# JamesYang007/adelie

Hardware: AMD Instinct MI355X
Metric: lambda-paths/sec (100-lambda grpnet); HBM GB/s vs peak (higher is better)
Workload: dtype f64

## Files before the change

### adelie_amd/_abi.py

```python
import ctypes as C
import os

import numpy as np

F32, F64 = 0, 1
COL_MAJOR, ROW_MAJOR = 0, 1
SCREEN_STRONG, SCREEN_PIVOT = 0, 1
GLM_GAUSSIAN, GLM_BINOMIAL_LOGIT, GLM_GAUSSIAN_IRLS, GLM_MULTINOMIAL, GLM_POISSON, GLM_BINOMIAL_PROBIT = 0, 1, 2, 3, 4, 5
GLM_CALLBACK = 6
GLM_COX = 7
TIE_BRESLOW, TIE_EFRON = 0, 1

POLL_FN = C.CFUNCTYPE(C.c_int, C.c_void_p, C.c_int, C.c_int64, C.c_void_p)
DONE_FN = C.CFUNCTYPE(None, C.c_int32, C.c_int, C.c_void_p)
GLM_GRADIENT_FN = C.CFUNCTYPE(C.c_int, C.c_void_p, C.c_void_p, C.c_void_p)
GLM_HESSIAN_FN = C.CFUNCTYPE(C.c_int, C.c_void_p, C.c_void_p, C.c_void_p, C.c_void_p, C.c_void_p)
GLM_LOSS_FN = C.CFUNCTYPE(C.c_int, C.c_void_p, C.c_void_p, C.POINTER(C.c_double))


CONS_SOLVE_FN = C.CFUNCTYPE(C.c_int, C.c_void_p, C.c_int64, C.c_int64, C.POINTER(C.c_double), C.POINTER(C.c_double),
                           C.POINTER(C.c_double), C.c_double, C.c_double, C.POINTER(C.c_double))
CONS_GRADIENT_FN = C.CFUNCTYPE(C.c_int, C.c_void_p, C.c_int64, C.c_int64, C.POINTER(C.c_double), C.POINTER(C.c_double))
CONS_SOLVE_ZERO_FN = C.CFUNCTYPE(C.c_int, C.c_void_p, C.c_int64, C.c_int64, C.POINTER(C.c_double), C.POINTER(C.c_double))
CONS_DUAL_FN = C.CFUNCTYPE(C.c_int, C.c_void_p, C.c_int64, C.c_int64, C.POINTER(C.c_double))
# ... 198 lines not shown
        + [(n, C.c_int64) for n in ("ns", "nv", "nblk", "n_list")]
        + [(n, C.c_void_p) for n in ("sbegin", "ssize", "voff", "blk_g0", "list", "desc", "Dblk", "gblk", "C")]
        + [("ldc", C.c_int64)]
        + [(n, C.c_void_p) for n in ("xmean", "spen", "vcol", "beta", "g", "is_active", "active_set")]
        + [(n, C.c_double) for n in ("l1", "l2", "newton_tol", "dbeta_tol")]
        + [(n, C.c_int64) for n in ("newton_max_iters", "max_active_size", "mark")]
        + [("rsq", C.c_double), ("resid_sum", C.c_double), ("n_updates", C.c_int64), ("active_size", C.c_int64)]
        + [(n, C.c_void_p) for n in ("dcol", "dlt", "dd", "st_f", "st_i")]
    )


(MULTI_SWEEP, MULTI_STEP, MULTI_FUSED_STEP, MULTI_BLOCK_LISTS, MULTI_EXPAND, MULTI_EXPAND_CROSS, MULTI_AXPY, MULTI_TO_MAJOR,
 MULTI_FROM_MAJOR, MULTI_BATCH_PICK) = range(10)


class MultiPiece(C.Structure):
    _fields_ = (
        [(n, C.c_int64) for n in ("dtype", "mode", "nb", "pb", "K", "icpt")]
        + [("X", C.c_void_p), ("X_elems", C.c_int64), ("x_off", C.c_int64), ("ld", C.c_int64), ("bits", C.c_void_p),
           ("bits_elems", C.c_int64), ("ldb", C.c_int64), ("impute", C.c_void_p), ("v", C.c_void_p), ("v_off", C.c_int64),
           ("out", C.c_void_p), ("w", C.c_void_p), ("r", C.c_void_p), ("dcol", C.c_void_p), ("dlt", C.c_void_p),
           ("n_dcol", C.c_int64), ("nz", C.c_int64), ("cols", C.c_void_p), ("nb_cols", C.c_int64), ("part", C.c_void_p),
           ("part_elems", C.c_int64), ("sign", C.c_double), ("nv", C.c_int64), ("nc", C.c_int64)]
        + [(n, C.c_void_p) for n in ("ulist", "slot", "resp", "slot_c", "resp_c", "C")]
        + [("C_elems", C.c_int64), ("ldc", C.c_int64), ("D", C.c_void_p), ("D_elems", C.c_int64), ("ldd", C.c_int64),
           ("lsel_list", C.c_void_p), ("n_lsel", C.c_int64), ("lsel", C.c_int64)]
    )


HIP_SYMBOLS = [
    "abi_version", "last_error", "device_count", "set_config",
    "design_create_dense", "design_create_sparse", "design_create_csc", "design_create_standardized", "design_adopt_dense_dev", "design_create_snp_unphased",
    "design_create_snp_calldata", "design_create_snp_bed", "design_alias", "design_drop_shadow", "design_shadow_stats", "design_shadow_info", "design_create_slice", "design_create_multi", "design_create_derived", "design_create_concat", "design_create_pieces", "design_impute", "design_destroy", "design_owned_bytes",
    "design_create_one_hot", "design_create_interaction", "design_factor_groups",
    "design_create_convex_relu", "design_create_convex_relu_csc",
    "design_create_snp_phased_ancestry", "design_create_snp_phased_calldata", "design_csc_download", "design_nnz",
    "design_glm_path_losses", "design_multi_path_losses", "design_cox_path_losses", "design_batch_stats", "design_rows", "design_cols", "design_dtype",
    "design_device", "design_stream",
    "design_cmul", "design_ctmul", "design_bmul", "design_btmul", "design_bmul_cols", "design_btmul_cols", "design_mul", "design_mul_batch", "design_cov",
    "design_sq_mul", "design_sp_tmul",
    "design_create_cov_dense", "design_create_cov_csc", "design_create_cov_lazy", "design_cov_bmul", "design_cov_mul", "design_cov_mul_batch", "design_cov_to_dense", "gaussian_cov_solve",
    "glm_cox_create", "glm_cox_destroy", "glm_cox_eval",
    "grpnet_solve", "grpnet_solve_many", "result_destroy", "result_size", "result_copy", "result_scalar", "result_error", "result_sync",
    "bench_sweep", "filter_sweep_test", "block_build_test", "group_piece_test", "multi_piece_test", "cov_piece_test",
    "css_cov_solve", "css_result_destroy", "css_result_size", "css_result_copy", "css_result_scalar", "css_result_error",
    "bvls_solve", "bvls_result_destroy", "bvls_result_size", "bvls_result_copy", "bvls_result_scalar", "bvls_result_error",
    "design_create_constraint_dense", "design_adopt_constraint_dense_dev", "design_create_constraint_csc", "constraint_op",
    "pinball_solve", "pinball_result_destroy", "pinball_result_size", "pinball_result_copy", "pinball_result_scalar",
    "pinball_result_error",
    "qp_full_solve",
]


def np_dtype(code):
    return np.float64 if code == F64 else np.float32


def dtype_code(dtype):
    dtype = np.dtype(dtype)
# ... 98 lines not shown
        sig("design_cov_bmul", ci, [vp, vp, i64, vp, vp, i64, vp])
        sig("design_cov_mul", ci, [vp, vp, vp, i64, vp])
        sig("design_cov_mul_batch", ci, [vp, i64, vp, vp, vp, vp, vp])
        sig("design_cov_to_dense", ci, [vp, i64, i64, vp])
        sig("result_destroy", ci, [vp])
        sig("result_size", i64, [vp, ci])
        sig("result_copy", ci, [vp, ci, vp, i64])
        sig("result_scalar", dbl, [vp, ci])
        sig("result_error", C.c_char_p, [vp])
        sig("result_sync", ci, [vp])
        sig("bench_sweep", ci, [vp, i64, p(dbl)])
        sig("filter_sweep_test", ci, [vp, vp, vp, dbl, vp, vp, i64, vp, vp, i64, vp, dbl, vp, vp, vp])
        sig("block_build_test", ci, [vp, ci, i64, vp, vp, i64, vp, i64, vp, ci, i64, ci, vp, i64, vp, i64, vp])
        sig("group_piece_test", ci, [p(GroupPiece), vp])
        sig("multi_piece_test", ci, [p(MultiPiece), vp])
        sig("cov_piece_test", ci, [vp, ci, vp, i64, i64, i64, i64, dbl, vp, vp, vp, i64, vp])
        sig("css_cov_solve", ci, [vp, p(CssArgs), p(vp)])
        sig("css_result_destroy", ci, [vp])
        sig("css_result_size", i64, [vp, ci])
        sig("css_result_copy", ci, [vp, ci, vp, i64])
        sig("css_result_scalar", dbl, [vp, ci])
        sig("css_result_error", C.c_char_p, [vp])
        sig("bvls_solve", ci, [vp, p(BvlsArgs), p(vp)])
        sig("bvls_result_destroy", ci, [vp])
        sig("bvls_result_size", i64, [vp, ci])
        sig("bvls_result_copy", ci, [vp, ci, vp, i64])
        sig("bvls_result_scalar", dbl, [vp, ci])
        sig("bvls_result_error", C.c_char_p, [vp])
        sig("design_create_constraint_dense", ci, [vp, i64, i64, ci, ci, ci, p(vp)])
        sig("design_adopt_constraint_dense_dev", ci, [vp, i64, i64, ci, ci, ci, p(vp)])
# ... 55 lines not shown
```

### adelie_amd/csrc/kernels.hpp

```cpp
#pragma once
#include <hip/hip_runtime.h>
#include <cstdint>
#include "gram_shape.hpp"
#include "multi_shape.hpp"
#include "relu_shape.hpp"
#include "relu_sparse_shape.hpp"
#include "shadow_kind_host.hpp"
#include "pieces_host.hpp"

namespace ahip {

template <class T>
struct DenseView {
    const T* X;
    int64_t n, p, ld;
};
struct SnpView {
    const uint8_t* bits;
    int64_t n, p, ldb;
};

template <class T>
struct PiecesView {
    const void* base[kMaxPieces];
// ... 443 lines not shown
int launch_panel_step(const DenseView<T>& X, const T* w, T* r, const int32_t* dcol, const T* dlt, const int32_t* nz_dev,
                      const int32_t* cols, int nb, T* part, hipStream_t s);
template <class T>
struct StepTail {
    int32_t* counter;
    int32_t base;
    T* g;
    const T* rsum;
    const T* xm;
};
template <class T>
int launch_panel_step_snp(const SnpView& X, const T* impute, const T* w, T* r, const int32_t* dcol, const T* dlt,
                          const int32_t* nz_dev, const int32_t* cols, int nb, T* part, hipStream_t s,
                          const StepTail<T>* tail = nullptr, bool* tailed = nullptr);
int64_t panel_part_elems(int64_t n);
template <class T>
void launch_la_open_from_grad(const T* grad, const int32_t* cols, int nb, T* g, const T* rsum_src, T* rsum_out, hipStream_t s);
template <class T>
void launch_panel_reduce(const T* part, int nslices, int nb, const int32_t* cols, const T* rsum_dev, const T* xm_by_col,
                         T* gblk, hipStream_t s);
template <class T>
void launch_panel_reduce_ld(const T* part, int64_t part_ld, int nslices, int nb, const int32_t* cols, const T* rsum_dev,
                            const T* xm_by_col, T* gblk, hipStream_t s);
template <class T>
int launch_panel_fused(const CdBlkParams<T>& sp, int j, const DenseView<T>& X, const T* w, T* r, const int32_t* dcol,
                       const T* dlt, const int32_t* nz_dev, const int32_t* cols, int nb, T* part, bool tr, hipStream_t s);
template <class T>
int launch_panel_fused_snp(const CdBlkParams<T>& sp, int j, const SnpView& X, const T* impute, const T* w, T* r,
                           const int32_t* dcol, const T* dlt, const int32_t* nz_dev, const int32_t* cols, int nb, T* part,
                           bool tr, hipStream_t s);
// ... 221 lines not shown
```

### adelie_amd/csrc/kernels_cd_panel.hip

```cpp
#include "kernels.hpp"
#include "accessors.hpp"
#include "wavered.hpp"
#include "blk_solve_body.hpp"
#include "grp_solve_body.hpp"

namespace ahip {

namespace {

constexpr int PB = 128;
constexpr int PT = 256;

template <class T, int VEC>
struct RawDense { Pack<T, VEC> v; };
struct RawSnp { unsigned byte; };

template <class T, int VEC>
__device__ __forceinline__ RawDense<T, VEC> praw(const DenseAcc<T>& X, int64_t j, int64_t i, int64_t n, bool full) {
    RawDense<T, VEC> r;
    const T* col = X.colptr(j);
    if constexpr (VEC == 1) {
        const T x = col[(full || i < n) ? i : 0];
        r.v.v[0] = (full || i < n) ? x : T(0);
    } else {
        using V = typename VecOf<T>::type;
        static_assert(VEC == VecOf<T>::N, "dense vector width");
// ... 24 lines not shown
template <class T, int VEC>
__device__ __forceinline__ Pack<T, VEC> pdecode(const SnpAcc<T>& X, const RawSnp& r, int64_t j, int64_t i, int64_t n) {
    Pack<T, VEC> o;
    const T imp = X.impute[j];
#pragma unroll
    for (int e = 0; e < VEC; ++e) {
        const unsigned c = (r.byte >> (2 * e)) & 3u;
        o.v[e] = (i + e < n) ? (c == 3u ? imp : T(c)) : T(0);
    }
    return o;
}
template <class T, class Acc, int VEC> struct RawOf;
template <class T, int VEC> struct RawOf<T, DenseAcc<T>, VEC> { using type = RawDense<T, VEC>; };
template <class T, int VEC> struct RawOf<T, SnpAcc<T>, VEC> { using type = RawSnp; };

template <class T, class Acc, int VEC, bool FULL, bool WGRED = false>
__device__ __forceinline__ void panel_step_body(const Acc& X, int64_t n, const T* __restrict__ w, T* __restrict__ r,
                                                const int32_t* __restrict__ dcol, const T* __restrict__ dlt, int nz,
                                                const int32_t* __restrict__ cols, int nb, T* __restrict__ part,
                                                int64_t part_ld, T (*red)[64 * VEC], T* wrs, int tid, int64_t slice) {
    constexpr int U = 16;
    using Raw = typename RawOf<T, Acc, VEC>::type;
    const int lane = tid & 63;
    const int wv = __builtin_amdgcn_readfirstlane(tid >> 6);
    const int64_t i = slice * (64 * VEC) + int64_t(lane) * VEC;
    const bool full = FULL ? true : (i + VEC <= n);

    constexpr int UB = 8;
    Raw xb[UB];
    int jb[UB];
    if (nb > 0) {
#pragma unroll
        for (int u = 0; u < UB; ++u) jb[u] = cols[min(wv + 4 * u, nb - 1)];
#pragma unroll
        for (int u = 0; u < UB; ++u) xb[u] = praw<T, VEC>(X, jb[u], i, n, full);
    }

    if (nz > 0) {
        T acc[VEC];
#pragma unroll
        for (int e = 0; e < VEC; ++e) acc[e] = T(0);
        for (int m0 = wv; m0 < nz; m0 += 4 * U) {
// ... 5 lines not shown
                const int m = m0 + 4 * u;
                ja[u] = dcol[min(m, nz - 1)];
                cf[u] = m < nz ? dlt[min(m, nz - 1)] : T(0);
            }
#pragma unroll
            for (int u = 0; u < U; ++u) xa[u] = praw<T, VEC>(X, ja[u], i, n, full);
#pragma unroll
            for (int u = 0; u < U; ++u) {
                const Pack<T, VEC> xx = pdecode<T, VEC>(X, xa[u], ja[u], i, n);
#pragma unroll
                for (int e = 0; e < VEC; ++e) acc[e] = fma(cf[u], xx.v[e], acc[e]);
            }
        }
#pragma unroll
        for (int e = 0; e < VEC; ++e) red[wv][lane * VEC + e] = acc[e];
        __syncthreads();
        if (wv == 0) {
#pragma unroll
            for (int e = 0; e < VEC; ++e) {
                const int q = lane * VEC + e;
                T wr = T(0);
                if (FULL || i + e < n) {
                    const T rr = r[i + e] - ((red[0][q] + red[1][q]) + (red[2][q] + red[3][q]));
                    r[i + e] = rr;
                    wr = w[i + e] * rr;
                }
                wrs[q] = wr;
            }
        }
    } else if (wv == 0) {
#pragma unroll
        for (int e = 0; e < VEC; ++e) wrs[lane * VEC + e] = (FULL || i + e < n) ? w[i + e] * r[i + e] : T(0);
    }
    if (nb <= 0) return;
    __syncthreads();

    T wr[VEC];
#pragma unroll
    for (int e = 0; e < VEC; ++e) wr[e] = wrs[lane * VEC + e];
    for (int c0 = wv; c0 < nb; c0 += 4 * UB) {
        if (c0 != wv) {
#pragma unroll
            for (int u = 0; u < UB; ++u) jb[u] = cols[min(c0 + 4 * u, nb - 1)];
#pragma unroll
            for (int u = 0; u < UB; ++u) xb[u] = praw<T, VEC>(X, jb[u], i, n, full);
        }
        T pu[UB];
#pragma unroll
        for (int u = 0; u < UB; ++u) {
            const Pack<T, VEC> xx = pdecode<T, VEC>(X, xb[u], jb[u], i, n);
            T sacc = T(0);
#pragma unroll
            for (int e = 0; e < VEC; ++e) sacc = fma(xx.v[e], wr[e], sacc);
            pu[u] = sacc;
        }
        static_assert(UB == 8, "reduce8");
        const T tot = reduce8(pu, lane);
        if (lane < UB && c0 + 4 * lane < nb) {
            if constexpr (WGRED) red[0][c0 + 4 * lane] = tot;
            else part[part_ld > 0 ? int64_t(c0 + 4 * lane) * part_ld + slice : slice * PB + (c0 + 4 * lane)] = tot;
        }
    }
}

template <class T, class Acc, int VEC>
__global__ __launch_bounds__(PT, (VEC >= 16 ? 2 : 4)) void panel_step_kernel(Acc X, int64_t n, const T* __restrict__ w, T* __restrict__ r,
                                                        const int32_t* __restrict__ dcol, const T* __restrict__ dlt,
                                                        const int32_t* __restrict__ nz_dev,
                                                        const int32_t* __restrict__ cols, int nb, T* __restrict__ part,
                                                        int64_t part_ld) {
    constexpr int RS = 64 * VEC;
    __shared__ T red[4][RS];
    __shared__ T wrs[RS];
    const int nz = nz_dev[0];
    if ((int64_t(blockIdx.x) + 1) * RS <= n)
        panel_step_body<T, Acc, VEC, true>(X, n, w, r, dcol, dlt, nz, cols, nb, part, part_ld, red, wrs, threadIdx.x, blockIdx.x);
    else
        panel_step_body<T, Acc, VEC, false>(X, n, w, r, dcol, dlt, nz, cols, nb, part, part_ld, red, wrs, threadIdx.x, blockIdx.x);
}

constexpr int S16_RS = 1024;
constexpr int S16_NSUB = 2;

template <class T>
__device__ __forceinline__ T reduce16(const T (&v)[16], int lane) {
    const bool b0 = lane & 1, b1 = lane & 2, b2 = lane & 4, b3 = lane & 8;
    T a[8], c[4], d[2];
#pragma unroll
    for (int m = 0; m < 8; ++m) {
        const T keep = b0 ? v[2 * m + 1] : v[2 * m], send = b0 ? v[2 * m] : v[2 * m + 1];
        a[m] = keep + pdpp<0xB1>(send);
    }
#pragma unroll
// ... 205 lines not shown
#pragma unroll
            for (int u = 0; u < 4; ++u)
                v[u] = (k0 + 64 * u < nwg) ? __hip_atomic_load(pc + k0 + 64 * u, __ATOMIC_RELAXED, __HIP_MEMORY_SCOPE_AGENT) : T(0);
#pragma unroll
            for (int u = 0; u < 4; ++u) sacc += v[u];
        }
        sacc = wave_sum64(sacc);
        if (lane == 0) {
            T g = sacc;
            if (tail.xm) g -= tail.rsum[0] * tail.xm[cols[c]];
            tail.g[c] = g;
        }
    }
}

constexpr int FS = 4;
template <class T>
constexpr size_t fused_lds() {
    return blk_solve_lds_la<T>() > size_t(148) * 1024 ? blk_solve_lds_la<T>() : size_t(148) * 1024;
}
template <class T, class Acc, int VEC>
__device__ __forceinline__ void fused_step_part(char* smem_raw, const Acc& X, int64_t n, const T* __restrict__ w,
                                                T* __restrict__ r, const int32_t* __restrict__ dcol,
                                                const T* __restrict__ dlt, const int32_t* __restrict__ nz_dev,
                                                const int32_t* __restrict__ cols, int nb, T* __restrict__ part,
                                                int64_t part_ld, int fsa, bool coh = false) {
    constexpr int RS = 64 * VEC;
    const int sub = threadIdx.x >> 8, tid = threadIdx.x & 255;
    T* base = reinterpret_cast<T*>(smem_raw) + size_t(sub) * 5 * RS;
    T (*red)[RS] = reinterpret_cast<T (*)[RS]>(base);
    T* wrs = base + 4 * RS;
    const int nz = nz_dev[0];
    static_assert(RS >= PB || VEC == 1, "a slice's LDS row holds the block's column partials");
    const int64_t grp = int64_t(blockIdx.x) - 1;
    const int64_t slice = grp * fsa + sub;
    if constexpr (RS >= PB) {
        if (sub >= fsa) {
            if (nz > 0) __syncthreads();
            if (nb <= 0) return;
            __syncthreads();
            if (tid < PB) red[0][tid] = T(0);
        } else if ((grp + 1) * fsa * RS <= n) {
            panel_step_body<T, Acc, VEC, true, true>(X, n, w, r, dcol, dlt, nz, cols, nb, part, part_ld, red, wrs, tid, slice);
        } else {
            panel_step_body<T, Acc, VEC, false, true>(X, n, w, r, dcol, dlt, nz, cols, nb, part, part_ld, red, wrs, tid, slice);
        }
        if (nb <= 0) return;
        __syncthreads();
        if (threadIdx.x < nb) {
            const T* b0 = reinterpret_cast<const T*>(smem_raw);
            const int c = threadIdx.x;
            const T tot = (b0[c] + b0[size_t(5) * RS + c]) + (b0[size_t(10) * RS + c] + b0[size_t(15) * RS + c]);
            T* dst = part + (part_ld > 0 ? int64_t(c) * part_ld + grp : grp * PB + c);
            if (coh) __hip_atomic_store(dst, tot, __ATOMIC_RELAXED, __HIP_MEMORY_SCOPE_AGENT);
            else *dst = tot;
        }
    } else {
        const int64_t slice4 = grp * FS + sub;
        if ((grp + 1) * FS * RS <= n)
            panel_step_body<T, Acc, VEC, true>(X, n, w, r, dcol, dlt, nz, cols, nb, part, part_ld, red, wrs, tid, slice4);
        else
            panel_step_body<T, Acc, VEC, false>(X, n, w, r, dcol, dlt, nz, cols, nb, part, part_ld, red, wrs, tid, slice4);
    }
}

inline int fused_fsa(int64_t ns) {
    if ((ns + 3) / 4 > 250) return 4;
    if (ns <= 250) return 1;
    if ((ns + 1) / 2 <= 250) return 2;
    return 4;
}

template <class T, class Acc, int VEC>
__global__ __launch_bounds__(256 * FS) void panel_fused_kernel(CdBlkParams<T> sp, int j, Acc X, int64_t n,
                                                              const T* __restrict__ w, T* __restrict__ r,
                                                              const int32_t* __restrict__ dcol, const T* __restrict__ dlt,
                                                              const int32_t* __restrict__ nz_dev,
                                                              const int32_t* __restrict__ cols, int nb,
                                                              T* __restrict__ part, int64_t part_ld, int fsa) {
    extern __shared__ __attribute__((aligned(16))) char smem_raw[];
    constexpr int RS = 64 * VEC;
    if (blockIdx.x == 0) {
        if (j < 0) {
            if (threadIdx.x == 0 && sp.part_rsum) {
                const T v = sp.part_rsum[0];
                sp.rsum_out[0] = v;
                sp.rsum_out[1] = v;
            }
            return;
        }
        blk_solve_la_body<T>(sp, j, smem_raw, threadIdx.x);
        return;
    }
    fused_step_part<T, Acc, VEC>(smem_raw, X, n, w, r, dcol, dlt, nz_dev, cols, nb, part, part_ld, fsa);
}

template <class T>
__global__ __launch_bounds__(PT) void panel_reduce_kernel(const T* __restrict__ part, int64_t part_ld, int nslices,
                                                          const int32_t* __restrict__ cols,
                                                          const T* __restrict__ rsum, const T* __restrict__ xm_by_col,
                                                          T* __restrict__ gblk) {
    __shared__ T red[4];
    const int c = blockIdx.x, tid = threadIdx.x, lane = tid & 63, wv = tid >> 6;
    const T* pc = part + int64_t(c) * part_ld;
    T s = T(0);
    for (int k = tid; k < nslices; k += PT) s += pc[k];
    s = wave_sum64(s);
    if (lane == 0) red[wv] = s;
    __syncthreads();
// ... 10 lines not shown
    if (a >= cnt) return;
    T v = vars[a];
    if (center) v -= xm[a] * xm[a];
    vars[a] = v > T(0) ? v : T(0);
}

__global__ void gather_i32_kernel(const int32_t* __restrict__ src, const int32_t* __restrict__ idx, int cnt,
                                  int32_t* __restrict__ out) {
    const int a = blockIdx.x * blockDim.x + threadIdx.x;
    if (a < cnt) out[a] = src[idx[a]];
}

template <class T, class Acc, int VEC>
int step_launch(const Acc& acc, int64_t n, const T* w, T* r, const int32_t* dcol, const T* dlt, const int32_t* nz_dev,
                const int32_t* cols, int nb, T* part, hipStream_t s) {
    constexpr int RS = 64 * VEC;
    const int64_t ns = (n + RS - 1) / RS;
    hipLaunchKernelGGL((panel_step_kernel<T, Acc, VEC>), dim3((unsigned)ns), dim3(PT), 0, s, acc, n, w, r, dcol, dlt,
                       nz_dev, cols, nb, part, ns);
    return int(ns);
}

template <class T, class Acc, int VEC>
__global__ __launch_bounds__(256 * FS) void panel_fused_grp_kernel(CdGrpBlkParams<T> sp, int j, Acc X, int64_t n,
                                                                  const T* __restrict__ w, T* __restrict__ r,
                                                                  const int32_t* __restrict__ dcol,
                                                                  const T* __restrict__ dlt,
                                                                  const int32_t* __restrict__ nz_dev,
                                                                  const int32_t* __restrict__ cols, int nb,
                                                                  T* __restrict__ part, int64_t part_ld, int fsa) {
    extern __shared__ __attribute__((aligned(16))) char smem_raw[];
    constexpr int RS = 64 * VEC;
// ... 52 lines not shown
            sp.tail_g[c] = g;
        }
        if (threadIdx.x == 0) {
            const int d = __hip_atomic_fetch_add(sp.tail_counter + 1, 1, __ATOMIC_RELAXED, __HIP_MEMORY_SCOPE_AGENT);
            if (d == NT - 1) {
                __hip_atomic_store(sp.tail_counter + 1, 0, __ATOMIC_RELAXED, __HIP_MEMORY_SCOPE_AGENT);
                __hip_atomic_store(sp.tail_counter, 0, __ATOMIC_RELAXED, __HIP_MEMORY_SCOPE_AGENT);
            }
        }
    }
}

template <class T, class Acc, int VEC>
int fused_grp_launch(const CdGrpBlkParams<T>& sp, int j, const Acc& acc, int64_t n, const T* w, T* r, const int32_t* dcol,
                     const T* dlt, const int32_t* nz_dev, const int32_t* cols, int nb, T* part, bool tr, hipStream_t s) {
    constexpr int RS = 64 * VEC;
    const int64_t ns = (n + RS - 1) / RS;
    const int fsa = (64 * VEC >= PB) ? fused_fsa(ns) : FS;
    const int64_t nwg = (ns + fsa - 1) / fsa;
    const int64_t part_ld = (64 * VEC >= PB) ? nwg : nwg * FS;
    static bool attr_done = false;
    if (!attr_done) {
        (void)hipFuncSetAttribute(reinterpret_cast<const void*>(panel_fused_grp_kernel<T, Acc, VEC>),
                                  hipFuncAttributeMaxDynamicSharedMemorySize, int(grp_solve_lds_total<T>()));
        attr_done = true;
    }
    hipLaunchKernelGGL((panel_fused_grp_kernel<T, Acc, VEC>), dim3((unsigned)(nwg + 1)), dim3(256 * FS),
                       grp_solve_lds_total<T>(), s, sp, j, acc, n, w, r, dcol, dlt, nz_dev, cols, nb, part,
                       tr ? int64_t(0) : part_ld, fsa);
    return int(part_ld);
}

template <class T, class Acc, int VEC>
int fused_launch(const CdBlkParams<T>& sp, int j, const Acc& acc, int64_t n, const T* w, T* r, const int32_t* dcol,
                 const T* dlt, const int32_t* nz_dev, const int32_t* cols, int nb, T* part, bool tr, hipStream_t s) {
    constexpr int RS = 64 * VEC;
    const int64_t ns = (n + RS - 1) / RS;
    const int fsa = (64 * VEC >= PB) ? fused_fsa(ns) : FS;
    const int64_t nwg = (ns + fsa - 1) / fsa;
    const int64_t part_ld = (64 * VEC >= PB) ? nwg : nwg * FS;
    static bool attr_done = false;
    if (!attr_done) {
        (void)hipFuncSetAttribute(reinterpret_cast<const void*>(panel_fused_kernel<T, Acc, VEC>),
                                  hipFuncAttributeMaxDynamicSharedMemorySize, int(fused_lds<T>()));
        attr_done = true;
    }
    hipLaunchKernelGGL((panel_fused_kernel<T, Acc, VEC>), dim3((unsigned)(nwg + 1)), dim3(256 * FS),
                       fused_lds<T>(), s, sp, j, acc, n, w, r, dcol, dlt, nz_dev, cols, nb, part,
                       tr ? int64_t(0) : part_ld, fsa);
    return int(part_ld);
}

}

template <class T>
int launch_panel_fused(const CdBlkParams<T>& sp, int j, const DenseView<T>& X, const T* w, T* r, const int32_t* dcol,
                       const T* dlt, const int32_t* nz_dev, const int32_t* cols, int nb, T* part, bool tr, hipStream_t s) {
    DenseAcc<T> acc{X.X, X.ld};
    constexpr int V = VecOf<T>::N;
    const bool vecok = (X.ld % V == 0) && ((reinterpret_cast<uintptr_t>(X.X) % 16) == 0);
    if (vecok) return fused_launch<T, DenseAcc<T>, V>(sp, j, acc, X.n, w, r, dcol, dlt, nz_dev, cols, nb, part, tr, s);
    return fused_launch<T, DenseAcc<T>, 1>(sp, j, acc, X.n, w, r, dcol, dlt, nz_dev, cols, nb, part, tr, s);
}
template <class T>
int launch_panel_fused_snp(const CdBlkParams<T>& sp, int j, const SnpView& X, const T* impute, const T* w, T* r,
                           const int32_t* dcol, const T* dlt, const int32_t* nz_dev, const int32_t* cols, int nb, T* part,
                           bool tr, hipStream_t s) {
    SnpAcc<T> acc{X.bits, X.ldb, impute};
    return fused_launch<T, SnpAcc<T>, 4>(sp, j, acc, X.n, w, r, dcol, dlt, nz_dev, cols, nb, part, tr, s);
}

template <class T>
int launch_panel_fused_grp(const CdGrpBlkParams<T>& sp, int j, const DenseView<T>& X, const T* w, T* r, const int32_t* dcol,
                           const T* dlt, const int32_t* nz_dev, const int32_t* cols, int nb, T* part, bool tr, hipStream_t s) {
    DenseAcc<T> acc{X.X, X.ld};
// ... 18 lines not shown
    if (c < nb) g[c] = grad[cols[c]];
    if (c == 0 && rsum_src) {
        const T v = rsum_src[0];
        rsum_out[0] = v;
        rsum_out[1] = v;
    }
}
}
template <class T>
void launch_la_open_from_grad(const T* grad, const int32_t* cols, int nb, T* g, const T* rsum_src, T* rsum_out, hipStream_t s) {
    hipLaunchKernelGGL((la_open_kernel<T>), dim3(1), dim3(PB), 0, s, grad, cols, nb, g, rsum_src, rsum_out);
}
template void launch_la_open_from_grad<double>(const double*, const int32_t*, int, double*, const double*, double*, hipStream_t);
template void launch_la_open_from_grad<float>(const float*, const int32_t*, int, float*, const float*, float*, hipStream_t);

int64_t panel_part_elems(int64_t n) { return int64_t(PB) * ((n + 63) / 64) + 16; }

template <class T>
int launch_panel_step(const DenseView<T>& X, const T* w, T* r, const int32_t* dcol, const T* dlt, const int32_t* nz_dev,
                      const int32_t* cols, int nb, T* part, hipStream_t s) {
    DenseAcc<T> acc{X.X, X.ld};
    constexpr int V = VecOf<T>::N;
    const bool vecok = (X.ld % V == 0) && ((reinterpret_cast<uintptr_t>(X.X) % 16) == 0);
    if (vecok) return step_launch<T, DenseAcc<T>, V>(acc, X.n, w, r, dcol, dlt, nz_dev, cols, nb, part, s);
    return step_launch<T, DenseAcc<T>, 1>(acc, X.n, w, r, dcol, dlt, nz_dev, cols, nb, part, s);
}

template <class T>
int launch_panel_step_snp(const SnpView& X, const T* impute, const T* w, T* r, const int32_t* dcol, const T* dlt,
                          const int32_t* nz_dev, const int32_t* cols, int nb, T* part, hipStream_t s, const StepTail<T>* tail,
                          bool* tailed) {
// ... 69 lines not shown
```

### adelie_amd/csrc/solver.hip

```cpp
#include "common.hpp"
#include "design_ops.hpp"
#include "filter_host.hpp"
#include "screen_reads_host.hpp"
#include "cox.hpp"

#include <algorithm>
#include <cstring>
#include <exception>
#include <type_traits>
#include <chrono>
#include <condition_variable>
#include <mutex>
#include <thread>
#include <cmath>
#include <cstdio>
#include <cstdlib>
#include <limits>
#include <numeric>
#include <unordered_set>

namespace ahip {
void set_last_error(const std::string& s);
double g_hessian_min = 1e-24;
double g_dbeta_tol = 1e-12;
// ... 1453 lines not shown
            up(dr, &scale, 1);
            if (a->w) up(dw, static_cast<const T*>(a->w), pb);
            launch_batch_pick<T>(dv.p, pb, int(K), int(a->lsel), dr.p, a->w ? dw.p : nullptr, dout.p, s);
            std::vector<T> h(static_cast<size_t>(pb));
            finish(a->out, h, dout.p);
        };
        if (a->dtype == ADELIE_HIP_F64) body(double{});
        else body(float{});
    } catch (const std::exception& e) {
        set_last_error(e.what());
        return 1;
    }
    return 0;
}

int adelie_hip_cov_piece_test(adelie_hip_design* A, int what, const int32_t* vcol, int64_t nv, int64_t pos0, int64_t N, int64_t ldc,
                              double sentinel, const void* v, const int32_t* cols, const void* coef, int64_t count, void* out) {
    try {
        if (!A || !out) throw make_core_error("bad arguments.");
        if (!A->cov) throw make_core_error("A must be a covariance matrix (matrix.dense(method=\"cov\")).");
        const int64_t p = A->p;
        const bool gather = what == ADELIE_HIP_COV_PIECE_GATHER;
        if (!gather && what != ADELIE_HIP_COV_PIECE_GRAD) throw make_core_error("unknown piece.");
        const int32_t* list = gather ? vcol : cols;
        const int64_t n_list = gather ? nv : count;
        if (gather && (!vcol || nv < 1 || nv > p || pos0 < 0 || N < 1 || pos0 + N != nv || ldc < nv || ldc > (int64_t(1) << 20)))
            throw make_core_error("GATHER: vcol (nv), 1 <= nv <= p, pos0 + N == nv and nv <= ldc are required.");
        if (!gather && (!v || count < 0 || count > p || (count > 0 && (!cols || !coef))))
            throw make_core_error("GRAD: v (p), cols and coef (count), 0 <= count <= p are required.");
        std::vector<uint8_t> seen(size_t(p), 0);
// ... 46 lines not shown
```

### include/adelie_hip.h

```cpp
#ifndef ADELIE_HIP_H
#define ADELIE_HIP_H

#include <stdint.h>

#ifdef __cplusplus
extern "C" {
#endif

#define ADELIE_HIP_ABI_VERSION 14

enum adelie_hip_dtype { ADELIE_HIP_F32 = 0, ADELIE_HIP_F64 = 1 };
enum adelie_hip_order { ADELIE_HIP_COL_MAJOR = 0, ADELIE_HIP_ROW_MAJOR = 1 };
enum adelie_hip_screen_rule { ADELIE_HIP_SCREEN_STRONG = 0, ADELIE_HIP_SCREEN_PIVOT = 1 };
enum adelie_hip_glm_kind {
    ADELIE_HIP_GLM_GAUSSIAN = 0,
    ADELIE_HIP_GLM_BINOMIAL_LOGIT = 1,
    ADELIE_HIP_GLM_GAUSSIAN_IRLS = 2,
    ADELIE_HIP_GLM_POISSON = 4,
    ADELIE_HIP_GLM_BINOMIAL_PROBIT = 5,
    ADELIE_HIP_GLM_CALLBACK = 6,
    ADELIE_HIP_GLM_COX = 7,
    ADELIE_HIP_GLM_MULTINOMIAL = 3
};

// ... 516 lines not shown
    int64_t nv, nc;
    int32_t* ulist;
    int32_t* slot;
    int32_t* resp;
    const int32_t* slot_c;
    const int32_t* resp_c;
    const void* C;
    int64_t C_elems, ldc;
    void* D;
    int64_t D_elems, ldd;
    const int64_t* lsel_list;
    int64_t n_lsel, lsel;
} adelie_hip_multi_piece;
int adelie_hip_multi_piece_test(const adelie_hip_multi_piece* a, int64_t* info);

enum adelie_hip_cov_piece { ADELIE_HIP_COV_PIECE_GATHER = 0, ADELIE_HIP_COV_PIECE_GRAD = 1 };
int adelie_hip_cov_piece_test(adelie_hip_design* A, int what, const int32_t* vcol, int64_t nv, int64_t pos0, int64_t N, int64_t ldc,
                              double sentinel, const void* v, const int32_t* cols, const void* coef, int64_t count, void* out);

enum adelie_hip_qp_full_kind { ADELIE_HIP_QP_FULL_NNQP = 0, ADELIE_HIP_QP_FULL_LASSO = 1, ADELIE_HIP_QP_FULL_PINBALL = 2 };
enum adelie_hip_qp_full_status { ADELIE_HIP_QP_FULL_OK = 0, ADELIE_HIP_QP_FULL_MAX_ITERS = 1 };
typedef struct adelie_hip_qp_full_args {
    int32_t            kind;
    int32_t            dtype;
    int32_t            device;
    int32_t            _pad0;
    int64_t            n_problems;
    const int64_t*     d;
    const void* const* quad;
    const uint8_t*     quad_is_dev;
// ... 18 lines not shown
```

Measured before the change: 5.015.

## Prefetch residual/weights and software-pipeline column loads in dense panel step kernels

For dense designs with vector width at least 2, the panel step body now loads r and w into registers before the reduction. It swaps __syncthreads for a bare LDS-wait plus s_barrier. When nb spans exactly four unroll rounds, it double-buffers column loads with scheduling barriers so global loads overlap the FMA reductions. It also moves the panel shape math into a shared header and adds a panel piece test entry point. The cost is higher register pressure and a special-case code path, and the lighter barrier relies on only LDS ordering being needed.

After: 5.039, median of 3. Within noise of the previous version (+0.5%).

```diff
diff --git a/adelie_amd/_abi.py b/adelie_amd/_abi.py
--- a/adelie_amd/_abi.py
+++ b/adelie_amd/_abi.py
@@ -236,6 +236,13 @@
  MULTI_FROM_MAJOR, MULTI_BATCH_PICK) = range(10)
 
 
+class PanelPiece(C.Structure):
+    _fields_ = [("mode", C.c_int64), ("d", C.c_void_p), ("row_off", C.c_int64), ("w", C.c_void_p), ("r", C.c_void_p),
+                ("dcol", C.c_void_p), ("dlt", C.c_void_p), ("n_dcol", C.c_int64), ("nz", C.c_int64), ("cols", C.c_void_p),
+                ("nb", C.c_int64), ("part", C.c_void_p), ("part_elems", C.c_int64), ("slice_major", C.c_int64), ("g", C.c_void_p),
+                ("g_elems", C.c_int64), ("xm", C.c_void_p), ("resid_sum", C.c_double)]
+
+
 class MultiPiece(C.Structure):
     _fields_ = (
         [(n, C.c_int64) for n in ("dtype", "mode", "nb", "pb", "K", "icpt")]
@@ -264,7 +271,7 @@
     "design_create_cov_dense", "design_create_cov_csc", "design_create_cov_lazy", "design_cov_bmul", "design_cov_mul", "design_cov_mul_batch", "design_cov_to_dense", "gaussian_cov_solve",
     "glm_cox_create", "glm_cox_destroy", "glm_cox_eval",
     "grpnet_solve", "grpnet_solve_many", "result_destroy", "result_size", "result_copy", "result_scalar", "result_error", "result_sync",
-    "bench_sweep", "filter_sweep_test", "block_build_test", "group_piece_test", "multi_piece_test", "cov_piece_test",
+    "bench_sweep", "filter_sweep_test", "block_build_test", "group_piece_test", "multi_piece_test", "panel_piece_test", "cov_piece_test",
     "css_cov_solve", "css_result_destroy", "css_result_size", "css_result_copy", "css_result_scalar", "css_result_error",
     "bvls_solve", "bvls_result_destroy", "bvls_result_size", "bvls_result_copy", "bvls_result_scalar", "bvls_result_error",
     "design_create_constraint_dense", "design_adopt_constraint_dense_dev", "design_create_constraint_csc", "constraint_op",
@@ -393,6 +400,7 @@
         sig("block_build_test", ci, [vp, ci, i64, vp, vp, i64, vp, i64, vp, ci, i64, ci, vp, i64, vp, i64, vp])
         sig("group_piece_test", ci, [p(GroupPiece), vp])
         sig("multi_piece_test", ci, [p(MultiPiece), vp])
+        sig("panel_piece_test", ci, [p(PanelPiece), vp])
         sig("cov_piece_test", ci, [vp, ci, vp, i64, i64, i64, i64, dbl, vp, vp, vp, i64, vp])
         sig("css_cov_solve", ci, [vp, p(CssArgs), p(vp)])
         sig("css_result_destroy", ci, [vp])
diff --git a/adelie_amd/csrc/kernels.hpp b/adelie_amd/csrc/kernels.hpp
--- a/adelie_amd/csrc/kernels.hpp
+++ b/adelie_amd/csrc/kernels.hpp
@@ -3,6 +3,7 @@
 #include <cstdint>
 #include "gram_shape.hpp"
 #include "multi_shape.hpp"
+#include "panel_shape.hpp"
 #include "relu_shape.hpp"
 #include "relu_sparse_shape.hpp"
 #include "shadow_kind_host.hpp"
@@ -481,6 +482,7 @@
                           const int32_t* nz_dev, const int32_t* cols, int nb, T* part, hipStream_t s,
                           const StepTail<T>* tail = nullptr, bool* tailed = nullptr);
 int64_t panel_part_elems(int64_t n);
+template <class T> int panel_step_vec(const DenseView<T>& X);
 template <class T>
 void launch_la_open_from_grad(const T* grad, const int32_t* cols, int nb, T* g, const T* rsum_src, T* rsum_out, hipStream_t s);
 template <class T>
diff --git a/adelie_amd/csrc/kernels_cd_panel.hip b/adelie_amd/csrc/kernels_cd_panel.hip
--- a/adelie_amd/csrc/kernels_cd_panel.hip
+++ b/adelie_amd/csrc/kernels_cd_panel.hip
@@ -1,15 +1,17 @@
 #include "kernels.hpp"
+#include <type_traits>
 #include "accessors.hpp"
 #include "wavered.hpp"
 #include "blk_solve_body.hpp"
 #include "grp_solve_body.hpp"
+#include "panel_shape.hpp"
 
 namespace ahip {
 
 namespace {
 
-constexpr int PB = 128;
-constexpr int PT = 256;
+constexpr int PB = kPanelB;
+constexpr int PT = kPanelThreads;
 
 template <class T, int VEC>
 struct RawDense { Pack<T, VEC> v; };
@@ -64,7 +66,9 @@
 template <class T, int VEC> struct RawOf<T, DenseAcc<T>, VEC> { using type = RawDense<T, VEC>; };
 template <class T, int VEC> struct RawOf<T, SnpAcc<T>, VEC> { using type = RawSnp; };
 
-template <class T, class Acc, int VEC, bool FULL, bool WGRED = false>
+__device__ __forceinline__ void lds_barrier() { asm volatile("s_waitcnt lgkmcnt(0)\n\ts_barrier" ::: "memory"); }
+
+template <class T, class Acc, int VEC, bool FULL, bool WGRED = false, bool STREAM = false>
 __device__ __forceinline__ void panel_step_body(const Acc& X, int64_t n, const T* __restrict__ w, T* __restrict__ r,
                                                 const int32_t* __restrict__ dcol, const T* __restrict__ dlt, int nz,
                                                 const int32_t* __restrict__ cols, int nb, T* __restrict__ part,
@@ -76,6 +80,17 @@
     const int64_t i = slice * (64 * VEC) + int64_t(lane) * VEC;
     const bool full = FULL ? true : (i + VEC <= n);
 
+    T rp[VEC], wp[VEC];
+    if constexpr (STREAM) {
+        if (wv == 0) {
+#pragma unroll
+            for (int e = 0; e < VEC; ++e) {
+                const int64_t q = (FULL || i + e < n) ? i + e : 0;
+                rp[e] = r[q];
+                wp[e] = w[q];
+            }
+        }
+    }
     constexpr int UB = 8;
     Raw xb[UB];
     int jb[UB];
@@ -111,41 +126,39 @@
         }
 #pragma unroll
         for (int e = 0; e < VEC; ++e) red[wv][lane * VEC + e] = acc[e];
-        __syncthreads();
+        if constexpr (STREAM) lds_barrier();
+        else __syncthreads();
         if (wv == 0) {
 #pragma unroll
             for (int e = 0; e < VEC; ++e) {
                 const int q = lane * VEC + e;
                 T wr = T(0);
                 if (FULL || i + e < n) {
-                    const T rr = r[i + e] - ((red[0][q] + red[1][q]) + (red[2][q] + red[3][q]));
+                    const T r0 = STREAM ? rp[e] : r[i + e];
+                    const T rr = r0 - ((red[0][q] + red[1][q]) + (red[2][q] + red[3][q]));
                     r[i + e] = rr;
-                    wr = w[i + e] * rr;
+                    wr = (STREAM ? wp[e] : w[i + e]) * rr;
                 }
                 wrs[q] = wr;
             }
         }
     } else if (wv == 0) {
 #pragma unroll
-        for (int e = 0; e < VEC; ++e) wrs[lane * VEC + e] = (FULL || i + e < n) ? w[i + e] * r[i + e] : T(0);
+        for (int e = 0; e < VEC; ++e)
+            wrs[lane * VEC + e] = (FULL || i + e < n) ? (STREAM ? wp[e] * rp[e] : w[i + e] * r[i + e]) : T(0);
     }
     if (nb <= 0) return;
-    __syncthreads();
+    if constexpr (STREAM) lds_barrier();
+    else __syncthreads();
 
     T wr[VEC];
 #pragma unroll
     for (int e = 0; e < VEC; ++e) wr[e] = wrs[lane * VEC + e];
-    for (int c0 = wv; c0 < nb; c0 += 4 * UB) {
-        if (c0 != wv) {
-#pragma unroll
-            for (int u = 0; u < UB; ++u) jb[u] = cols[min(c0 + 4 * u, nb - 1)];
-#pragma unroll
-            for (int u = 0; u < UB; ++u) xb[u] = praw<T, VEC>(X, jb[u], i, n, full);
-        }
+    const auto consume = [&](const Raw(&x)[UB], const int(&j)[UB], int c0) {
         T pu[UB];
 #pragma unroll
         for (int u = 0; u < UB; ++u) {
-            const Pack<T, VEC> xx = pdecode<T, VEC>(X, xb[u], jb[u], i, n);
+            const Pack<T, VEC> xx = pdecode<T, VEC>(X, x[u], j[u], i, n);
             T sacc = T(0);
 #pragma unroll
             for (int e = 0; e < VEC; ++e) sacc = fma(xx.v[e], wr[e], sacc);
@@ -157,6 +170,43 @@
             if constexpr (WGRED) red[0][c0 + 4 * lane] = tot;
             else part[part_ld > 0 ? int64_t(c0 + 4 * lane) * part_ld + slice : slice * PB + (c0 + 4 * lane)] = tot;
         }
+    };
+    if constexpr (STREAM) {
+        if (wv + 3 * 4 * UB < nb && wv + 4 * 4 * UB >= nb) {
+            Raw x1[UB];
+            int j1[UB], j2[UB], j3[UB];
+#pragma unroll
+            for (int u = 0; u < UB; ++u) {
+                j1[u] = cols[min(wv + 4 * UB + 4 * u, nb - 1)];
+                j2[u] = cols[min(wv + 8 * UB + 4 * u, nb - 1)];
+                j3[u] = cols[min(wv + 12 * UB + 4 * u, nb - 1)];
+            }
+#pragma unroll
+            for (int u = 0; u < UB; ++u) x1[u] = praw<T, VEC>(X, j1[u], i, n, full);
+            __builtin_amdgcn_sched_barrier(0);
+            consume(xb, jb, wv);
+            __builtin_amdgcn_sched_barrier(0);
+#pragma unroll
+            for (int u = 0; u < UB; ++u) xb[u] = praw<T, VEC>(X, j2[u], i, n, full);
+            __builtin_amdgcn_sched_barrier(0);
+            consume(x1, j1, wv + 4 * UB);
+            __builtin_amdgcn_sched_barrier(0);
+#pragma unroll
+            for (int u = 0; u < UB; ++u) x1[u] = praw<T, VEC>(X, j3[u], i, n, full);
+            __builtin_amdgcn_sched_barrier(0);
+            consume(xb, j2, wv + 8 * UB);
+            consume(x1, j3, wv + 12 * UB);
+            return;
+        }
+    }
+    for (int c0 = wv; c0 < nb; c0 += 4 * UB) {
+        if (c0 != wv) {
+#pragma unroll
+            for (int u = 0; u < UB; ++u) jb[u] = cols[min(c0 + 4 * u, nb - 1)];
+#pragma unroll
+            for (int u = 0; u < UB; ++u) xb[u] = praw<T, VEC>(X, jb[u], i, n, full);
+        }
+        consume(xb, jb, c0);
     }
 }
 
@@ -169,11 +219,19 @@
     constexpr int RS = 64 * VEC;
     __shared__ T red[4][RS];
     __shared__ T wrs[RS];
-    const int nz = nz_dev[0];
-    if ((int64_t(blockIdx.x) + 1) * RS <= n)
-        panel_step_body<T, Acc, VEC, true>(X, n, w, r, dcol, dlt, nz, cols, nb, part, part_ld, red, wrs, threadIdx.x, blockIdx.x);
-    else
-        panel_step_body<T, Acc, VEC, false>(X, n, w, r, dcol, dlt, nz, cols, nb, part, part_ld, red, wrs, threadIdx.x, blockIdx.x);
+    if constexpr (std::is_same<Acc, DenseAcc<T>>::value && VEC >= 2) {
+        const int nz = nz_dev[0];
+        if ((int64_t(blockIdx.x) + 1) * RS <= n)
+            panel_step_body<T, Acc, VEC, true, false, true>(X, n, w, r, dcol, dlt, nz, cols, nb, part, part_ld, red, wrs, threadIdx.x, blockIdx.x);
+        else
+            panel_step_body<T, Acc, VEC, false, false, true>(X, n, w, r, dcol, dlt, nz, cols, nb, part, part_ld, red, wrs, threadIdx.x, blockIdx.x);
+    } else {
+        const int nz = nz_dev[0];
+        if ((int64_t(blockIdx.x) + 1) * RS <= n)
+            panel_step_body<T, Acc, VEC, true>(X, n, w, r, dcol, dlt, nz, cols, nb, part, part_ld, red, wrs, threadIdx.x, blockIdx.x);
+        else
+            panel_step_body<T, Acc, VEC, false>(X, n, w, r, dcol, dlt, nz, cols, nb, part, part_ld, red, wrs, threadIdx.x, blockIdx.x);
+    }
 }
 
 constexpr int S16_RS = 1024;
@@ -409,12 +467,12 @@
     }
 }
 
-constexpr int FS = 4;
+constexpr int FS = kPanelFS;
 template <class T>
 constexpr size_t fused_lds() {
     return blk_solve_lds_la<T>() > size_t(148) * 1024 ? blk_solve_lds_la<T>() : size_t(148) * 1024;
 }
-template <class T, class Acc, int VEC>
+template <class T, class Acc, int VEC, bool STREAM = false>
 __device__ __forceinline__ void fused_step_part(char* smem_raw, const Acc& X, int64_t n, const T* __restrict__ w,
                                                 T* __restrict__ r, const int32_t* __restrict__ dcol,
                                                 const T* __restrict__ dlt, const int32_t* __restrict__ nz_dev,
@@ -436,9 +494,15 @@
             __syncthreads();
             if (tid < PB) red[0][tid] = T(0);
         } else if ((grp + 1) * fsa * RS <= n) {
-            panel_step_body<T, Acc, VEC, true, true>(X, n, w, r, dcol, dlt, nz, cols, nb, part, part_ld, red, wrs, tid, slice);
+            if constexpr (STREAM && std::is_same<Acc, DenseAcc<T>>::value)
+                panel_step_body<T, Acc, VEC, true, true, true>(X, n, w, r, dcol, dlt, nz, cols, nb, part, part_ld, red, wrs, tid, slice);
+            else
+                panel_step_body<T, Acc, VEC, true, true>(X, n, w, r, dcol, dlt, nz, cols, nb, part, part_ld, red, wrs, tid, slice);
         } else {
-            panel_step_body<T, Acc, VEC, false, true>(X, n, w, r, dcol, dlt, nz, cols, nb, part, part_ld, red, wrs, tid, slice);
+            if constexpr (STREAM && std::is_same<Acc, DenseAcc<T>>::value)
+                panel_step_body<T, Acc, VEC, false, true, true>(X, n, w, r, dcol, dlt, nz, cols, nb, part, part_ld, red, wrs, tid, slice);
+            else
+                panel_step_body<T, Acc, VEC, false, true>(X, n, w, r, dcol, dlt, nz, cols, nb, part, part_ld, red, wrs, tid, slice);
         }
         if (nb <= 0) return;
         __syncthreads();
@@ -457,13 +521,6 @@
         else
             panel_step_body<T, Acc, VEC, false>(X, n, w, r, dcol, dlt, nz, cols, nb, part, part_ld, red, wrs, tid, slice4);
     }
-}
-
-inline int fused_fsa(int64_t ns) {
-    if ((ns + 3) / 4 > 250) return 4;
-    if (ns <= 250) return 1;
-    if ((ns + 1) / 2 <= 250) return 2;
-    return 4;
 }
 
 template <class T, class Acc, int VEC>
@@ -487,7 +544,7 @@
         blk_solve_la_body<T>(sp, j, smem_raw, threadIdx.x);
         return;
     }
-    fused_step_part<T, Acc, VEC>(smem_raw, X, n, w, r, dcol, dlt, nz_dev, cols, nb, part, part_ld, fsa);
+    fused_step_part<T, Acc, VEC, true>(smem_raw, X, n, w, r, dcol, dlt, nz_dev, cols, nb, part, part_ld, fsa);
 }
 
 template <class T>
@@ -528,8 +585,7 @@
 template <class T, class Acc, int VEC>
 int step_launch(const Acc& acc, int64_t n, const T* w, T* r, const int32_t* dcol, const T* dlt, const int32_t* nz_dev,
                 const int32_t* cols, int nb, T* part, hipStream_t s) {
-    constexpr int RS = 64 * VEC;
-    const int64_t ns = (n + RS - 1) / RS;
+    const int64_t ns = panel_step_shape(n, VEC).slices;
     hipLaunchKernelGGL((panel_step_kernel<T, Acc, VEC>), dim3((unsigned)ns), dim3(PT), 0, s, acc, n, w, r, dcol, dlt,
                        nz_dev, cols, nb, part, ns);
     return int(ns);
@@ -612,11 +668,9 @@
 template <class T, class Acc, int VEC>
 int fused_grp_launch(const CdGrpBlkParams<T>& sp, int j, const Acc& acc, int64_t n, const T* w, T* r, const int32_t* dcol,
                      const T* dlt, const int32_t* nz_dev, const int32_t* cols, int nb, T* part, bool tr, hipStream_t s) {
-    constexpr int RS = 64 * VEC;
-    const int64_t ns = (n + RS - 1) / RS;
-    const int fsa = (64 * VEC >= PB) ? fused_fsa(ns) : FS;
-    const int64_t nwg = (ns + fsa - 1) / fsa;
-    const int64_t part_ld = (64 * VEC >= PB) ? nwg : nwg * FS;
+    const PanelStepShape sh = panel_fused_shape(n, VEC);
+    const int fsa = sh.fsa;
+    const int64_t nwg = sh.wgs, part_ld = sh.part_n;
     static bool attr_done = false;
     if (!attr_done) {
         (void)hipFuncSetAttribute(reinterpret_cast<const void*>(panel_fused_grp_kernel<T, Acc, VEC>),
@@ -632,11 +686,9 @@
 template <class T, class Acc, int VEC>
 int fused_launch(const CdBlkParams<T>& sp, int j, const Acc& acc, int64_t n, const T* w, T* r, const int32_t* dcol,
                  const T* dlt, const int32_t* nz_dev, const int32_t* cols, int nb, T* part, bool tr, hipStream_t s) {
-    constexpr int RS = 64 * VEC;
-    const int64_t ns = (n + RS - 1) / RS;
-    const int fsa = (64 * VEC >= PB) ? fused_fsa(ns) : FS;
-    const int64_t nwg = (ns + fsa - 1) / fsa;
-    const int64_t part_ld = (64 * VEC >= PB) ? nwg : nwg * FS;
+    const PanelStepShape sh = panel_fused_shape(n, VEC);
+    const int fsa = sh.fsa;
+    const int64_t nwg = sh.wgs, part_ld = sh.part_n;
     static bool attr_done = false;
     if (!attr_done) {
         (void)hipFuncSetAttribute(reinterpret_cast<const void*>(panel_fused_kernel<T, Acc, VEC>),
@@ -652,11 +704,19 @@
 }
 
 template <class T>
+int panel_step_vec(const DenseView<T>& X) {
+    constexpr int V = VecOf<T>::N;
+    return ((X.ld % V == 0) && ((reinterpret_cast<uintptr_t>(X.X) % 16) == 0)) ? V : 1;
+}
+template int panel_step_vec<double>(const DenseView<double>&);
+template int panel_step_vec<float>(const DenseView<float>&);
+
+template <class T>
 int launch_panel_fused(const CdBlkParams<T>& sp, int j, const DenseView<T>& X, const T* w, T* r, const int32_t* dcol,
                        const T* dlt, const int32_t* nz_dev, const int32_t* cols, int nb, T* part, bool tr, hipStream_t s) {
     DenseAcc<T> acc{X.X, X.ld};
     constexpr int V = VecOf<T>::N;
-    const bool vecok = (X.ld % V == 0) && ((reinterpret_cast<uintptr_t>(X.X) % 16) == 0);
+    const bool vecok = panel_step_vec<T>(X) == V;
     if (vecok) return fused_launch<T, DenseAcc<T>, V>(sp, j, acc, X.n, w, r, dcol, dlt, nz_dev, cols, nb, part, tr, s);
     return fused_launch<T, DenseAcc<T>, 1>(sp, j, acc, X.n, w, r, dcol, dlt, nz_dev, cols, nb, part, tr, s);
 }
@@ -705,7 +765,7 @@
 template void launch_la_open_from_grad<double>(const double*, const int32_t*, int, double*, const double*, double*, hipStream_t);
 template void launch_la_open_from_grad<float>(const float*, const int32_t*, int, float*, const float*, float*, hipStream_t);
 
-int64_t panel_part_elems(int64_t n) { return int64_t(PB) * ((n + 63) / 64) + 16; }
+int64_t panel_part_elems(int64_t n) { return panel_part_elems_for(n); }
 
 template <class T>
 int launch_panel_step(const DenseView<T>& X, const T* w, T* r, const int32_t* dcol, const T* dlt, const int32_t* nz_dev,
diff --git a/adelie_amd/csrc/panel_shape.hpp b/adelie_amd/csrc/panel_shape.hpp
--- /dev/null
+++ b/adelie_amd/csrc/panel_shape.hpp
@@ -0,0 +1,58 @@
+#pragma once
+#include <cstdint>
+
+namespace ahip {
+
+constexpr int kPanelB = 128;
+constexpr int kPanelThreads = 256;
+constexpr int kPanelFS = 4;
+
+inline int64_t panel_slice_rows(int vec) { return int64_t(64) * vec; }
+inline int64_t panel_slices(int64_t n, int vec) { return (n + panel_slice_rows(vec) - 1) / panel_slice_rows(vec); }
+
+inline int fused_fsa(int64_t ns) {
+    if ((ns + 3) / 4 > 250) return 4;
+    if (ns <= 250) return 1;
+    if ((ns + 1) / 2 <= 250) return 2;
+    return 4;
+}
+
+struct PanelStepShape {
+    int vec;
+    int64_t slices;
+    int fsa;
+    int64_t wgs;
+    int64_t part_n;
+    bool wgred;
+};
+
+inline PanelStepShape panel_step_shape(int64_t n, int vec) {
+    PanelStepShape s{};
+    s.vec = vec;
+    s.slices = panel_slices(n, vec);
+    s.fsa = 1;
+    s.wgs = s.slices;
+    s.part_n = s.slices;
+    s.wgred = false;
+    return s;
+}
+
+inline PanelStepShape panel_fused_shape(int64_t n, int vec) {
+    PanelStepShape s{};
+    s.vec = vec;
+    s.slices = panel_slices(n, vec);
+    s.wgred = 64 * vec >= kPanelB;
+    s.fsa = s.wgred ? fused_fsa(s.slices) : kPanelFS;
+    s.wgs = (s.slices + s.fsa - 1) / s.fsa;
+    s.part_n = s.wgred ? s.wgs : s.wgs * kPanelFS;
+    return s;
+}
+
+inline int64_t panel_part_elems_for(int64_t n) { return int64_t(kPanelB) * ((n + 63) / 64) + 16; }
+
+inline int64_t panel_part_extent(const PanelStepShape& s, int nb, bool slice_major) {
+    if (nb <= 0 || s.part_n <= 0) return 0;
+    return slice_major ? (s.part_n - 1) * kPanelB + nb : int64_t(nb) * s.part_n;
+}
+
+}
diff --git a/adelie_amd/csrc/solver.hip b/adelie_amd/csrc/solver.hip
--- a/adelie_amd/csrc/solver.hip
+++ b/adelie_amd/csrc/solver.hip
@@ -1491,6 +1491,135 @@
     return 0;
 }
 
+int adelie_hip_panel_piece_test(const adelie_hip_panel_piece* a, int64_t* info) {
+    try {
+        if (!a || !info || !a->d) throw make_core_error("bad arguments.");
+        adelie_hip_design* d = a->d;
+        if (d->cov || d->constraint || d->std_center || d->is_multi() || !d->is_dense()) throw make_core_error("a plain dense design is required.");
+        no_pieces(*d, "adelie_hip_panel_piece_test");
+        const int mode = int(a->mode);
+        if (a->mode < ADELIE_HIP_PANEL_STEP || a->mode > ADELIE_HIP_PANEL_FUSED_STEP) throw make_core_error("unknown mode.");
+        constexpr int64_t G = kPanelB;
+        if (a->row_off < 0 || a->row_off >= d->n) throw make_core_error("0 <= row_off < n is required.");
+        const int64_t n = d->n - a->row_off, p = d->p;
+        if (!a->w || !a->r || !a->part || !a->g) throw make_core_error("w, r, part and g are required.");
+        if (a->n_dcol < 0 || a->n_dcol > G || a->nz < 0 || a->nz > a->n_dcol || (a->n_dcol > 0 && (!a->dcol || !a->dlt)))
+            throw make_core_error("0 <= nz <= n_dcol <= 128 with dcol and dlt is required.");
+        if (a->nb < 0 || a->nb > G || (a->nb > 0 && !a->cols)) throw make_core_error("0 <= nb <= 128 with cols is required.");
+        for (int64_t m = 0; m < a->n_dcol; ++m)
+            if (a->dcol[m] < 0 || a->dcol[m] >= p) throw make_core_error("dcol: column out of range.");
+        for (int64_t c = 0; c < a->nb; ++c)
+            if (a->cols[c] < 0 || a->cols[c] >= p) throw make_core_error("cols: column out of range.");
+        if (a->slice_major != 0 && a->slice_major != 1) throw make_core_error("slice_major is 0 or 1.");
+        const bool fused = mode != ADELIE_HIP_PANEL_STEP;
+        const bool sm = fused && a->slice_major != 0;
+        if (!fused && a->slice_major) throw make_core_error("STEP leaves column-major partials.");
+        if (a->part_elems < 1 || a->part_elems > (int64_t(1) << 28) || a->g_elems < std::max<int64_t>(a->nb, 1) || a->g_elems > (1 << 20))
+            throw make_core_error("bad output shape.");
+        AHIP_CHECK(hipSetDevice(d->device));
+        hipStream_t s = d->stream;
+        for (int q = 0; q < 8; ++q) info[q] = 0;
+        auto body = [&](auto tag) {
+            using T = decltype(tag);
+            DenseView<T> Xd = d->dense<T>();
+            Xd.X += a->row_off;
+            Xd.n = n;
+            const int vec = panel_step_vec<T>(Xd);
+            const PanelStepShape sh = fused ? panel_fused_shape(n, vec) : panel_step_shape(n, vec);
+            const int nb = int(a->nb);
+            if (panel_part_extent(sh, nb, sm) > a->part_elems) throw make_core_error("part holds fewer elements than the launch writes.");
+            auto up = [&](auto& buf, const auto* h, int64_t cnt) { buf.reserve(size_t(cnt)); buf.upload(h, size_t(cnt), s); };
+            auto down = [&](void* h, const void* dev, size_t bytes) { AHIP_CHECK(hipMemcpyAsync(h, dev, bytes, hipMemcpyDeviceToHost, s)); };
+            DevBuf<T> dw, dr, ddlt, dpart, dg, dxm, drsum;
+            DevBuf<int32_t> ddcol, dcols, dnz;
+            up(dw, static_cast<const T*>(a->w), n);
+            up(dr, static_cast<const T*>(a->r), n);
+            ddcol.reserve(size_t(G)); ddlt.reserve(size_t(G)); dcols.reserve(size_t(G));
+            AHIP_CHECK(hipMemsetAsync(ddcol.p, 0, size_t(G) * sizeof(int32_t), s));
+            AHIP_CHECK(hipMemsetAsync(ddlt.p, 0, size_t(G) * sizeof(T), s));
+            AHIP_CHECK(hipMemsetAsync(dcols.p, 0, size_t(G) * sizeof(int32_t), s));
+            if (a->n_dcol > 0) {
+                ddcol.upload(a->dcol, size_t(a->n_dcol), s);
+                ddlt.upload(static_cast<const T*>(a->dlt), size_t(a->n_dcol), s);
+            }
+            if (nb > 0) dcols.upload(a->cols, size_t(nb), s);
+            const int32_t nz32 = int32_t(a->nz);
+            up(dnz, &nz32, 1);
+            up(dpart, static_cast<const T*>(a->part), a->part_elems);
+            up(dg, static_cast<const T*>(a->g), a->g_elems);
+            if (a->xm) up(dxm, static_cast<const T*>(a->xm), p);
+            const T rs = T(a->resid_sum);
+            up(drsum, &rs, 1);
+            const T* xmp = a->xm ? dxm.p : nullptr;
+            int got = 0, launches = 0;
+            DevBuf<T> dvars, dxmean, dspen, dbeta, dgb, dDb, dsdlt, dsdd;
+            DevBuf<int32_t> dvcol, dact, dsdcol;
+            DevBuf<int8_t> disact;
+            DevBuf<CdBlkState<T>> dst;
+            if (!fused) {
+                got = launch_panel_step<T>(Xd, dw.p, dr.p, ddcol.p, ddlt.p, dnz.p, dcols.p, nb, dpart.p, s);
+                ++launches;
+            } else {
+                CdBlkParams<T> bp{};
+                int j = -1;
+                if (mode == ADELIE_HIP_PANEL_FUSED_STEP) {
+                    const T one = T(1), zero = T(0);
+                    const int32_t zero32 = 0;
+                    const int8_t zero8 = 0;
+                    up(dvars, &one, 1); up(dxmean, &zero, 1); up(dspen, &one, 1); up(dbeta, &zero, 1); up(dvcol, &zero32, 1);
+                    up(disact, &zero8, 1);
+                    dact.reserve(4);
+                    AHIP_CHECK(hipMemsetAsync(dact.p, 0, 4 * sizeof(int32_t), s));
+                    CdBlkState<T> st0{};
+                    up(dst, &st0, 1);
+                    dDb.reserve(size_t(G * G)); dgb.reserve(size_t(G)); dsdlt.reserve(size_t(G)); dsdd.reserve(size_t(G)); dsdcol.reserve(size_t(G));
+                    AHIP_CHECK(hipMemsetAsync(dDb.p, 0, size_t(G * G) * sizeof(T), s));
+                    AHIP_CHECK(hipMemsetAsync(dgb.p, 0, size_t(G) * sizeof(T), s));
+                    AHIP_CHECK(hipMemsetAsync(dsdlt.p, 0, size_t(G) * sizeof(T), s));
+                    AHIP_CHECK(hipMemsetAsync(dsdd.p, 0, size_t(G) * sizeof(T), s));
+                    AHIP_CHECK(hipMemsetAsync(dsdcol.p, 0, size_t(G) * sizeof(int32_t), s));
+                    bp.nv = 1; bp.vars = dvars.p; bp.xmean = dxmean.p; bp.spen = dspen.p; bp.beta = dbeta.p;
+                    bp.is_active = disact.p; bp.active_set = dact.p; bp.l1 = T(1); bp.l2 = T(0); bp.max_active_size = 1;
+                    bp.st = dst.p; bp.list = nullptr; bp.count = 1; bp.mark = 0; bp.bsz = int32_t(G);
+                    bp.report_j = -1; bp.gblk = dgb.p; bp.Dptr = dDb.p; bp.vcol = dvcol.p; bp.dcol = dsdcol.p; bp.dlt = dsdlt.p;
+                    bp.dd = dsdd.p;
+                    j = 0;
+                }
+                got = launch_panel_fused<T>(bp, j, Xd, dw.p, dr.p, ddcol.p, ddlt.p, dnz.p, dcols.p, nb, dpart.p, sm, s);
+                ++launches;
+            }
+            AHIP_CHECK(hipGetLastError());
+            if (got != sh.part_n) throw make_core_error("the launcher's partial count differs from the shape header's.");
+            if (!sm && nb > 0) {
+                if (fused) launch_panel_reduce_ld<T>(dpart.p, sh.part_n, int(sh.part_n), nb, dcols.p, drsum.p, xmp, dg.p, s);
+                else launch_panel_reduce<T>(dpart.p, int(sh.part_n), nb, dcols.p, drsum.p, xmp, dg.p, s);
+                ++launches;
+                AHIP_CHECK(hipGetLastError());
+            }
+            std::vector<T> hr(static_cast<size_t>(n)), hp(static_cast<size_t>(a->part_elems)), hg(static_cast<size_t>(a->g_elems));
+            CdBlkState<T> hst{};
+            down(hr.data(), dr.p, hr.size() * sizeof(T));
+            down(hp.data(), dpart.p, hp.size() * sizeof(T));
+            down(hg.data(), dg.p, hg.size() * sizeof(T));
+            if (mode == ADELIE_HIP_PANEL_FUSED_STEP) down(&hst, dst.p, sizeof(hst));
+            AHIP_CHECK(hipStreamSynchronize(s));
+            if (mode == ADELIE_HIP_PANEL_FUSED_STEP && (hst.nz != 0 || hst.n_updates != 0 || hst.status != 0))
+                throw make_core_error("FUSED_STEP: the solve beside the step changed something.");
+            std::memcpy(a->r, hr.data(), hr.size() * sizeof(T));
+            std::memcpy(a->part, hp.data(), hp.size() * sizeof(T));
+            std::memcpy(a->g, hg.data(), hg.size() * sizeof(T));
+            info[0] = sh.vec; info[1] = sh.slices; info[2] = sh.fsa; info[3] = sh.wgs; info[4] = sh.part_n; info[5] = sm ? 1 : 0;
+            info[6] = launches;
+        };
+        if (d->dtype == ADELIE_HIP_F64) body(double{});
+        else body(float{});
+    } catch (const std::exception& e) {
+        set_last_error(e.what());
+        return 1;
+    }
+    return 0;
+}
+
 int adelie_hip_cov_piece_test(adelie_hip_design* A, int what, const int32_t* vcol, int64_t nv, int64_t pos0, int64_t N, int64_t ldc,
                               double sentinel, const void* v, const int32_t* cols, const void* coef, int64_t count, void* out) {
     try {
diff --git a/include/adelie_hip.h b/include/adelie_hip.h
--- a/include/adelie_hip.h
+++ b/include/adelie_hip.h
@@ -554,6 +554,27 @@
 } adelie_hip_multi_piece;
 int adelie_hip_multi_piece_test(const adelie_hip_multi_piece* a, int64_t* info);
 
+enum adelie_hip_panel_piece_mode { ADELIE_HIP_PANEL_STEP = 0, ADELIE_HIP_PANEL_FUSED_OPEN = 1, ADELIE_HIP_PANEL_FUSED_STEP = 2 };
+typedef struct adelie_hip_panel_piece {
+    int64_t mode;
+    adelie_hip_design* d;
+    int64_t row_off;
+    const void* w;
+    void* r;
+    const int32_t* dcol;
+    const void* dlt;
+    int64_t n_dcol, nz;
+    const int32_t* cols;
+    int64_t nb;
+    void* part;
+    int64_t part_elems, slice_major;
+    void* g;
+    int64_t g_elems;
+    const void* xm;
+    double resid_sum;
+} adelie_hip_panel_piece;
+int adelie_hip_panel_piece_test(const adelie_hip_panel_piece* a, int64_t* info);
+
 enum adelie_hip_cov_piece { ADELIE_HIP_COV_PIECE_GATHER = 0, ADELIE_HIP_COV_PIECE_GRAD = 1 };
 int adelie_hip_cov_piece_test(adelie_hip_design* A, int what, const int32_t* vcol, int64_t nv, int64_t pos0, int64_t N, int64_t ldc,
                               double sentinel, const void* v, const int32_t* cols, const void* coef, int64_t count, void* out);
```
